# stella-cv/stella_vslam

Hardware: AMD Instinct MI355X
Metric: frames/s ORB-extract+match @640x480,2k kpts (higher is better)
Workload: dtype u8

## Files before the change

stella_vslam_amd/csrc/orb_kernels.hip:

```cpp
#include "svgpu_internal.h"
#include <cstdlib>
#include <utility>

#pragma clang fp contract(off)

namespace {

__device__ __constant__ float c_pattern_f[1024] = {
#include "orb_pattern_i8.inc"
};

__device__ __forceinline__ int find_level(const OrbLevel* __restrict__ L, int num_levels, int idx, int OrbLevel::*first,
                                          int* local) {
    int lv = 0;
    for (int l = 0; l < num_levels; ++l) {
        const int f = L[l].*first;
        if (idx >= f) lv = l;
    }
    *local = idx - L[lv].*first;
    return lv;
}

__device__ __forceinline__ int reflect101(int p, int len) {
    if (len == 1) return 0;
    while (p < 0 || p >= len) p = p < 0 ? -p : 2 * (len - 1) - p;
    return p;
}

typedef unsigned short u16x2 __attribute__((ext_vector_type(2)));
__device__ __forceinline__ u16x2 as_u16x2(uint32_t v) { return __builtin_bit_cast(u16x2, v); }

__device__ __forceinline__ void xcd_frame_map(int per_frame, int batch, int& item, int& frame) {
    const int lin = blockIdx.x + blockIdx.y * gridDim.x;
    const int full = (batch / 8) * 8, lim = full * per_frame;
    if (lin < lim) {
        const int xcd = lin & 7, idx = lin >> 3;
        frame = (idx / per_frame) * 8 + xcd;
        item = idx % per_frame;
    }
    else {
        const int r = lin - lim;
        frame = full + r / per_frame;
        item = r % per_frame;
    }
}

__device__ __forceinline__ void sv_glds16(unsigned long long base, uint32_t voff, uint32_t lds_dst) {
    uint32_t keep;
    asm volatile("s_mov_b32 %0, m0\n\ts_mov_b32 m0, %3\n\ts_nop 2\n\tglobal_load_lds_dwordx4 %1, %2\n\ts_mov_b32 m0, %0"
                 : "=&s"(keep)
                 : "v"(voff), "s"(base), "s"(lds_dst)
                 : "memory");
}

__global__ __launch_bounds__(256) void k_resize(const uint8_t* __restrict__ src, size_t src_frame_stride, int src_pitch,
                                                int sw, uint8_t* __restrict__ dst, size_t dst_frame_stride, int dst_pitch,
                                                int dw, int dh, const short* __restrict__ xofs,
                                                const short2* __restrict__ xa, const short2* __restrict__ yofs,
                                                const short2* __restrict__ yb) {
    const int dy = blockIdx.y * 4 + threadIdx.y;
    const int dx0 = (blockIdx.x * 64 + threadIdx.x) * 4;
    if (dy >= dh || dx0 >= dw) return;
    const uint8_t* S = src + (size_t)blockIdx.z * src_frame_stride;
    const short2 yo = yofs[dy];
    const short2 bb = yb[dy];
    const uint8_t* S0 = S + (size_t)yo.x * src_pitch;
    const uint8_t* S1 = S + (size_t)yo.y * src_pitch;
    uint32_t packed = 0;
#pragma unroll
    for (int i = 0; i < 4; ++i) {
        const int dx = dx0 + i;
        if (dx < dw) {
            const int sx = xofs[dx];
            const short2 a = xa[dx];
            const int sx1 = min(sx + 1, sw - 1);
            const int r0 = S0[sx] * a.x + S0[sx1] * a.y;
            const int r1 = S1[sx] * a.x + S1[sx1] * a.y;
            const int v = ((((int)bb.x * (r0 >> 4)) >> 16) + (((int)bb.y * (r1 >> 4)) >> 16) + 2) >> 2;
            packed |= (uint32_t)(v & 255) << (8 * i);
        }
    }
    uint8_t* D = dst + (size_t)blockIdx.z * dst_frame_stride + (size_t)dy * dst_pitch + dx0;
    *reinterpret_cast<uint32_t*>(D) = packed;
}

#define PYR_THREADS 1024
#define PYR_MAXW 4096
__global__ __launch_bounds__(PYR_THREADS) void k_pyramid(const OrbLevel* __restrict__ L, int num_levels, const int2* __restrict__ band_rows,
                                                         const uint8_t* __restrict__ img0, size_t img0_frame_stride, int img0_pitch,
                                                         uint8_t* __restrict__ pyr, size_t pyr_frame_bytes,
                                                         const short* __restrict__ xofs, const short2* __restrict__ xa,
                                                         const short2* __restrict__ yofs, const short2* __restrict__ yb) {
    __shared__ short s_xo[PYR_MAXW];
    __shared__ short2 s_xa[PYR_MAXW];
    const int band = blockIdx.x, b = blockIdx.y, tid = threadIdx.x;
    uint8_t* P = pyr + (size_t)b * pyr_frame_bytes;
    for (int l = 1; l < num_levels; ++l) {
        const OrbLevel lev = L[l], prev = L[l - 1];
        const uint8_t* S = l == 1 ? img0 + (size_t)b * img0_frame_stride : P + prev.pyr_off;
        const int sp = l == 1 ? img0_pitch : prev.pitch;
        uint8_t* Dst = P + lev.pyr_off;
        const int2 rr = band_rows[band * num_levels + l];
        const int groups = (lev.w + 3) >> 2, ntask = (rr.y - rr.x) * groups;
        const bool in_lds = lev.w <= PYR_MAXW;
        if (in_lds)
            for (int x = tid; x < lev.w; x += PYR_THREADS) {
                s_xo[x] = xofs[lev.xtab_off + x];
                s_xa[x] = xa[lev.xtab_off + x];
            }
        __syncthreads();
        for (int t = tid; t < ntask; t += PYR_THREADS) {
            const int row = t / groups, g = t - row * groups;
            const int dy = rr.x + row, dx0 = g * 4;
            const short2 yo = yofs[lev.ytab_off + dy], bb = yb[lev.ytab_off + dy];
            const uint8_t* S0 = S + (size_t)yo.x * sp;
            const uint8_t* S1 = S + (size_t)yo.y * sp;
            int sx[4], sx1[4];
            short2 a[4];
#pragma unroll
            for (int i = 0; i < 4; ++i) {
                const int dx = min(dx0 + i, lev.w - 1);
                sx[i] = in_lds ? s_xo[dx] : xofs[lev.xtab_off + dx];
                a[i] = in_lds ? s_xa[dx] : xa[lev.xtab_off + dx];
                sx1[i] = min(sx[i] + 1, prev.w - 1);
            }
            int p00[4], p01[4], p10[4], p11[4];
#pragma unroll
            for (int i = 0; i < 4; ++i) {
                p00[i] = S0[sx[i]];
                p01[i] = S0[sx1[i]];
                p10[i] = S1[sx[i]];
                p11[i] = S1[sx1[i]];
            }
            uint32_t packed = 0;
#pragma unroll
            for (int i = 0; i < 4; ++i) {
                const int r0 = p00[i] * a[i].x + p01[i] * a[i].y;
                const int r1 = p10[i] * a[i].x + p11[i] * a[i].y;
                const int v = ((((int)bb.x * (r0 >> 4)) >> 16) + (((int)bb.y * (r1 >> 4)) >> 16) + 2) >> 2;
                packed |= (uint32_t)(v & 255) << (8 * i);
            }
            *reinterpret_cast<uint32_t*>(Dst + (size_t)dy * lev.pitch + dx0) = packed;
        }
        __syncthreads();
    }
}

__device__ __forceinline__ uint32_t mul_hi_u24(uint32_t a, uint32_t b) {
    uint32_t d;
    asm("v_mul_hi_u32_u24 %0, %1, %2" : "=v"(d) : "v"(a), "v"(b));
    return d;
}

__global__ __launch_bounds__(PYR_THREADS) void k_pyramid_lds(const OrbLevel* __restrict__ L, int num_levels, const int2* __restrict__ band_rows,
                                                             int bands, const uint8_t* __restrict__ img0, size_t img0_frame_stride,
                                                             int img0_pitch, uint8_t* __restrict__ pyr, size_t pyr_frame_bytes,
                                                             const uint32_t* __restrict__ xg, const short4* __restrict__ yrow) {
    extern __shared__ __attribute__((aligned(16))) uint8_t s_mem[];
    __shared__ int s_img[SV_MAX_LEVELS], s_yt[SV_MAX_LEVELS + 1];
    const int band = blockIdx.x, b = blockIdx.y, tid = threadIdx.x;
    const int2* BR = band_rows + (size_t)band * num_levels;
    if (tid == 0) {
        int size_a = 0, size_b = 0;
        for (int l = 0; l < num_levels; ++l) {
            const int bytes = (BR[l].y - BR[l].x) * ((L[l].w + 3) & ~3);
            if (l & 1) size_a = max(size_a, bytes);
            else size_b = max(size_b, bytes);
        }
        size_a = (size_a + 15) & ~15;
        size_b = (size_b + 15) & ~15;
        for (int l = 0; l < num_levels; ++l) s_img[l] = (l & 1) ? 0 : size_a;
        int off = size_a + size_b;
        s_yt[0] = off;
        for (int l = 1; l < num_levels; ++l) {
            s_yt[l] = off;
            off += (BR[l].y - BR[l].x) * 8;
        }
        s_yt[num_levels] = off;
    }
    __syncthreads();
    const uint8_t* I0 = img0 + (size_t)b * img0_frame_stride;
    {
        const int w0 = L[0].w, p0 = (w0 + 3) & ~3, lo0 = BR[0].x, n0 = BR[0].y - lo0;
        uint8_t* D0 = s_mem + s_img[0];
        if (((((size_t)I0) | (size_t)img0_pitch) & 15) == 0 && (p0 & 15) == 0) {
            const int cpr = p0 >> 4, total = n0 * cpr;
            const float inv = 1.0f / (float)cpr;
            for (int i = tid; i < total; i += PYR_THREADS) {
                const int r = (int)(((float)i + 0.5f) * inv), c = i - __mul24(r, cpr);
                reinterpret_cast<uint4*>(D0)[i] = *reinterpret_cast<const uint4*>(I0 + (__umul24(lo0 + r, img0_pitch) + 16 * c));
            }
        }
        else if (((((size_t)I0) | (size_t)img0_pitch) & 3) == 0) {
            const int wpr = p0 >> 2, total = n0 * wpr;
            const float inv = 1.0f / (float)wpr;
            for (int i = tid; i < total; i += PYR_THREADS) {
                const int r = (int)(((float)i + 0.5f) * inv), c = i - __mul24(r, wpr);
                reinterpret_cast<uint32_t*>(D0)[i] = *reinterpret_cast<const uint32_t*>(I0 + (__umul24(lo0 + r, img0_pitch) + 4 * c));
            }
        }
        else {
            const int total = n0 * p0;
            for (int i = tid; i < total; i += PYR_THREADS) {
                const int r = i / p0, c = i - r * p0;
                D0[i] = c < w0 ? I0[(size_t)(lo0 + r) * img0_pitch + c] : (uint8_t)0;
            }
        }
        const int rows = (s_yt[num_levels] - s_yt[0]) >> 3;
        for (int i = tid; i < rows; i += PYR_THREADS) {
            int l = 1;
            while (l + 1 < num_levels && s_yt[0] + 8 * i >= s_yt[l + 1]) ++l;
            const int r = i - ((s_yt[l] - s_yt[0]) >> 3);
            reinterpret_cast<short4*>(s_mem + s_yt[0])[i] = yrow[L[l].ytab_off + BR[l].x + r];
        }
    }
    __syncthreads();
    uint8_t* P = pyr + (size_t)b * pyr_frame_bytes;
    for (int l = 1; l < num_levels; ++l) {
        const OrbLevel lev = L[l];
        const int spw = ((L[l - 1].w + 3) & ~3) >> 2, dpw = ((lev.w + 3) & ~3) >> 2;
        const int src_lo = BR[l - 1].x, lo = BR[l].x, hi = BR[l].y;
        const int own_lo = (int)((long long)band * lev.h / bands), own_hi = (int)((long long)(band + 1) * lev.h / bands);
        const uint32_t* S = reinterpret_cast<const uint32_t*>(s_mem + s_img[l - 1]);
        uint32_t* Dl = reinterpret_cast<uint32_t*>(s_mem + s_img[l]);
        const short4* yt = reinterpret_cast<const short4*>(s_mem + s_yt[l]);
        uint8_t* Dg = P + lev.pyr_off;
        const int groups = (lev.w + 3) >> 2, nrows = hi - lo;
        const int chunks = max(min(PYR_THREADS / groups, nrows), 1), rc = (nrows + chunks - 1) / chunks;
        const int c = (int)(((float)tid + 0.5f) * (1.0f / (float)groups)), g = tid - __mul24(c, groups);
        const int r0 = __mul24(c, rc), r1 = min(r0 + rc, nrows);
        if (r0 < r1) {
            const uint4 e = reinterpret_cast<const uint4*>(xg)[2 * (lev.xg_off + g)];
            const uint2 e2 = reinterpret_cast<const uint2*>(xg)[4 * (lev.xg_off + g) + 2];
            const int i0 = e.x & 0xffff, i2 = e.x >> 16;
            const uint32_t coef[4] = {e.z, e.w, e2.x, e2.y};
            uint32_t sel[4];
#pragma unroll
            for (int i = 0; i < 4; ++i) sel[i] = 0x0c010c00u + ((e.y >> (8 * i)) & 255u) * 0x00010001u;
            const uint32_t* S0 = S + (i0 - __mul24(src_lo, spw));
            const int d2 = i2 - i0;
            auto hrow = [&](int sy, uint32_t (&h)[4]) {
                const uint32_t* R = S0 + __mul24(sy, spw);
                const uint32_t a0 = R[0], a1 = R[1], c0 = R[d2], c1 = R[d2 + 1];
                h[0] = __builtin_amdgcn_udot2(as_u16x2(__builtin_amdgcn_perm(a1, a0, sel[0])), as_u16x2(coef[0]), 0u, false) & ~15u;
                h[1] = __builtin_amdgcn_udot2(as_u16x2(__builtin_amdgcn_perm(a1, a0, sel[1])), as_u16x2(coef[1]), 0u, false) & ~15u;
                h[2] = __builtin_amdgcn_udot2(as_u16x2(__builtin_amdgcn_perm(c1, c0, sel[2])), as_u16x2(coef[2]), 0u, false) & ~15u;
                h[3] = __builtin_amdgcn_udot2(as_u16x2(__builtin_amdgcn_perm(c1, c0, sel[3])), as_u16x2(coef[3]), 0u, false) & ~15u;
            };
            uint32_t* dl = Dl + (__mul24(r0, dpw) + g);
            uint32_t goff = __umul24(lo + r0, lev.pitch) + 4 * g;
            const uint32_t own_n = (uint32_t)(own_hi - own_lo);
            uint32_t dyo = (uint32_t)(lo + r0 - own_lo);
            int prev = -1;
            auto step = [&](int row, uint32_t (&top)[4], uint32_t (&bot)[4]) {
                const short4 ye = yt[row];
                if (ye.x != prev) hrow(ye.x, top);
                hrow(ye.y, bot);
                prev = ye.y;
                const uint32_t b0 = (uint32_t)ye.z << 12, b1 = (uint32_t)ye.w << 12;
                uint32_t v[4];
#pragma unroll
                for (int i = 0; i < 4; ++i) v[i] = (mul_hi_u24(b0, top[i]) + mul_hi_u24(b1, bot[i]) + 2u) >> 2;
                const uint32_t packed = (v[0] & 255u) | ((v[1] & 255u) << 8) | ((v[2] & 255u) << 16) | (v[3] << 24);
                *dl = packed;
                if (dyo < own_n) *reinterpret_cast<uint32_t*>(Dg + goff) = packed;
                dl += dpw;
                goff += (uint32_t)lev.pitch;
                ++dyo;
            };
            uint32_t hX[4], hY[4] = {0, 0, 0, 0};
            int row = r0;
            for (; row + 1 < r1; row += 2) {
                step(row, hY, hX);
                step(row + 1, hX, hY);
            }
            if (row < r1) step(row, hY, hX);
        }
        __syncthreads();
    }
}

#define BLUR_EDGE_ROWS 8
struct BlurRow {
    uint32_t w0, w1, w2;
};
enum { BLUR_INTERIOR = 0, BLUR_EDGE = 1, BLUR_GATHER = 2, BLUR_LDS = 3 };
struct BlurEdge {
    bool left, hi_p1;
    uint32_t sel1, sel2;
};
__device__ __forceinline__ uint32_t blur_selector(int xbase, int lo_base, int w) {
    uint32_t s = 0;
#pragma unroll
    for (int k = 0; k < 4; ++k) {
        const int x = xbase + k, sx = x < w ? x : 2 * (w - 1) - x;
        s |= (uint32_t)min(max(sx - lo_base, 0), 7) << (8 * k);
    }
    return s;
}
__device__ __forceinline__ BlurEdge blur_edge_ctx(int x0, int w) {
    BlurEdge e;
    e.left = x0 == 0;
    e.hi_p1 = x0 + 4 < w;
    e.sel1 = blur_selector(x0, x0 - 4, w);
    e.sel2 = blur_selector(x0 + 4, e.hi_p1 ? x0 : x0 - 4, w);
    return e;
}
template <int MODE>
__device__ __forceinline__ BlurRow blur_load(const uint8_t* __restrict__ row, int x0, int w, const BlurEdge& e) {
    BlurRow r;
    if (MODE == BLUR_INTERIOR) {
        const uint32_t* p = reinterpret_cast<const uint32_t*>(row + x0 - 4);
        r.w0 = p[0];
        r.w1 = p[1];
        r.w2 = p[2];
    }
    else if (MODE == BLUR_EDGE) {
        if (e.left) {
            const uint32_t* p = reinterpret_cast<const uint32_t*>(row);
            r.w1 = p[0];
            r.w2 = p[1];
            r.w0 = __builtin_amdgcn_perm(r.w2, r.w1, 0x01020304u);
        }
        else {
            const uint32_t* p = reinterpret_cast<const uint32_t*>(row + x0 - 4);
            const uint32_t pm1 = p[0], p0 = p[1], p1 = e.hi_p1 ? p[2] : 0u;
            r.w0 = pm1;
            r.w1 = __builtin_amdgcn_perm(p0, pm1, e.sel1);
            r.w2 = e.hi_p1 ? __builtin_amdgcn_perm(p1, p0, e.sel2) : __builtin_amdgcn_perm(p0, pm1, e.sel2);
        }
    }
    else {
        uint32_t b[12];
#pragma unroll
        for (int k = 0; k < 12; ++k) b[k] = row[reflect101(x0 - 4 + k, w)];
        r.w0 = b[0] | (b[1] << 8) | (b[2] << 16) | (b[3] << 24);
        r.w1 = b[4] | (b[5] << 8) | (b[6] << 16) | (b[7] << 24);
        r.w2 = b[8] | (b[9] << 8) | (b[10] << 16) | (b[11] << 24);
    }
    return r;
}
__device__ __forceinline__ void blur_hpair(const BlurRow& a, const BlurRow& b, u16x2 (&hp)[4]) {
    u16x2 q[10];
#define SV_PK(WA, WB, K) as_u16x2(__builtin_amdgcn_perm(WB, WA, 0x0c000c00u | ((4u + K) << 16) | K))
    q[0] = SV_PK(a.w0, b.w0, 1u);
    q[1] = SV_PK(a.w0, b.w0, 2u);
    q[2] = SV_PK(a.w0, b.w0, 3u);
    q[3] = SV_PK(a.w1, b.w1, 0u);
    q[4] = SV_PK(a.w1, b.w1, 1u);
    q[5] = SV_PK(a.w1, b.w1, 2u);
    q[6] = SV_PK(a.w1, b.w1, 3u);
    q[7] = SV_PK(a.w2, b.w2, 0u);
    q[8] = SV_PK(a.w2, b.w2, 1u);
    q[9] = SV_PK(a.w2, b.w2, 2u);
#undef SV_PK
    const u16x2 t18 = {18, 18}, t34 = {34, 34}, t48 = {48, 48}, t56 = {56, 56};
#pragma unroll
    for (int j = 0; j < 4; ++j) hp[j] = t18 * (q[j] + q[j + 6]) + t34 * (q[j + 1] + q[j + 5]) + t48 * (q[j + 2] + q[j + 4]) + t56 * q[j + 3];
}
__device__ __forceinline__ uint32_t blur_dot(u16x2 h, uint32_t taps, uint32_t acc) { return __builtin_amdgcn_udot2(h, as_u16x2(taps), acc, false); }
__device__ __forceinline__ uint32_t blur_pack(const uint32_t (&acc)[4]) {
    const uint32_t lo = __builtin_amdgcn_perm(acc[1], acc[0], 0x0c0c0602u), hi = __builtin_amdgcn_perm(acc[3], acc[2], 0x06020c0cu);
    return lo | hi;
}

template <int MODE, class LoadPair>
__device__ __forceinline__ void blur_walk(LoadPair load_pair, uint8_t* __restrict__ Dp, int dpitch, int ys, int ye) {
    constexpr int AHEAD = MODE == BLUR_LDS ? 0 : 2;
    u16x2 A[4], B[4], C[4], D[4], E[4];
    BlurRow n0 = {}, n1 = {};
    {
        BlurRow r[8];
#pragma unroll
        for (int k = 0; k < 4; ++k) load_pair(ys - 4 + 2 * k, r[2 * k], r[2 * k + 1]);
        if (AHEAD) load_pair(ys + 4, n0, n1);
        if (MODE == BLUR_INTERIOR) {
#pragma unroll
            for (int k = 0; k < 8; ++k) asm volatile("" : "+v"(r[k].w0), "+v"(r[k].w1), "+v"(r[k].w2));
            asm volatile("" : "+v"(n0.w0), "+v"(n0.w1), "+v"(n0.w2), "+v"(n1.w0), "+v"(n1.w1), "+v"(n1.w2));
        }
        blur_hpair(r[0], r[1], A);
        blur_hpair(r[2], r[3], B);
        blur_hpair(r[4], r[5], C);
        blur_hpair(r[6], r[7], D);
    }
    for (int y = ys; y < ye; y += 2) {
        const BlurRow c0 = n0, c1 = n1;
        load_pair(y + 4 + AHEAD, n0, n1);
        if (AHEAD) blur_hpair(c0, c1, E);
        else blur_hpair(n0, n1, E);
        uint32_t acc[4];
#pragma unroll
        for (int j = 0; j < 4; ++j)
            acc[j] = blur_dot(D[j], 34u | (18u << 16), blur_dot(C[j], 56u | (48u << 16), blur_dot(B[j], 34u | (48u << 16), blur_dot(A[j], 18u << 16, 32768u))));
        *reinterpret_cast<uint32_t*>(Dp + __umul24(y, dpitch)) = blur_pack(acc);
        if (y + 1 < ye) {
#pragma unroll
            for (int j = 0; j < 4; ++j)
                acc[j] = blur_dot(E[j], 18u, blur_dot(D[j], 48u | (34u << 16), blur_dot(C[j], 48u | (56u << 16), blur_dot(B[j], 18u | (34u << 16), 32768u))));
            *reinterpret_cast<uint32_t*>(Dp + __umul24(y + 1, dpitch)) = blur_pack(acc);
        }
#pragma unroll
        for (int j = 0; j < 4; ++j) {
            A[j] = B[j];
            B[j] = C[j];
            C[j] = D[j];
            D[j] = E[j];
        }
    }
}
template <int MODE>
__device__ __forceinline__ void blur_strip(const uint8_t* __restrict__ src, int spitch, int w, int h, uint8_t* __restrict__ dst,
                                           int dpitch, int x0, int ys, int ye) {
    auto row_ptr = [&](int y) { return src + __umul24(reflect101(y, h), spitch); };
    BlurEdge edge = {};
    if (MODE == BLUR_EDGE) edge = blur_edge_ctx(x0, w);
    blur_walk<MODE>([&](int y, BlurRow& a, BlurRow& b) {
        a = blur_load<MODE>(row_ptr(y), x0, w, edge);
        b = blur_load<MODE>(row_ptr(y + 1), x0, w, edge);
    }, dst + x0, dpitch, ys, ye);
}

__device__ __forceinline__ void blur_locate(const OrbLevel* __restrict__ L, int num_levels, const uint8_t* __restrict__ img0,
                                            size_t img0_frame_stride, int img0_pitch, const uint8_t* __restrict__ pyr,
                                            size_t pyr_frame_bytes, uint8_t* __restrict__ blur, size_t blur_frame_bytes, OrbLevel& lev,
                                            int& tile, const uint8_t*& src, int& spitch, uint8_t*& dst,
                                            int OrbLevel::*first = &OrbLevel::btile_first) {
    int b, item;
    xcd_frame_map(gridDim.x, gridDim.y, item, b);
    const int lv = find_level(L, num_levels, item, first, &tile);
    lev = L[lv];
    if (lv == 0) {
        src = img0 + (size_t)b * img0_frame_stride;
        spitch = img0_pitch;
    }
    else {
        src = pyr + (size_t)b * pyr_frame_bytes + lev.pyr_off;
        spitch = lev.pitch;
    }
    dst = blur + (size_t)b * blur_frame_bytes + lev.blur_off;
}
__device__ __forceinline__ bool blur_streamable(const uint8_t* src, int spitch, int w) {
    return ((((size_t)src) | (size_t)spitch) & 3) == 0 && w >= 16;
}
template <int ROWS>
__global__ __launch_bounds__(256) void k_blur(const OrbLevel* __restrict__ L, int num_levels, const uint8_t* __restrict__ img0,
                                              size_t img0_frame_stride, int img0_pitch, const uint8_t* __restrict__ pyr,
                                              size_t pyr_frame_bytes, uint8_t* __restrict__ blur, size_t blur_frame_bytes) {
    OrbLevel lev;
    int tile, spitch;
    const uint8_t* src;
    uint8_t* dst;
    blur_locate(L, num_levels, img0, img0_frame_stride, img0_pitch, pyr, pyr_frame_bytes, blur, blur_frame_bytes, lev, tile, src, spitch, dst);
    if (!blur_streamable(src, spitch, lev.w)) return;
    const int main_tiles = lev.btiles_x * lev.btiles_y;
    if (tile < main_tiles) {
        const int tx = tile % lev.btiles_x, ty = tile / lev.btiles_x;
        const int rem_groups = tx == lev.btiles_x - 1 ? (min(lev.w - 6, (tx + 1) * BLUR_TW) - tx * BLUR_TW + 3) / 4 : 64;
        int g = 64;
        while (g > 1 && (g >> 1) >= rem_groups) g >>= 1;
        if (g <= 32 && rem_groups > 0) {
            const int spw = 64 / g, lane = threadIdx.x & 63;
            if (ty * spw >= lev.btiles_y) return;
            const int strip = (ty * 4 + (int)(threadIdx.x >> 6)) * spw + lane / g;
            const int x0 = tx * BLUR_TW + (lane % g) * 4, ys = strip * ROWS;
            if (x0 >= lev.w || ys >= lev.h) return;
            if (x0 >= 4 && x0 + 6 < lev.w) blur_strip<BLUR_INTERIOR>(src, spitch, lev.w, lev.h, dst, lev.pitch, x0, ys, min(ys + ROWS, lev.h));
            return;
        }
        const int x0 = tx * BLUR_TW + (threadIdx.x & 63) * 4;
        const int ys = __builtin_amdgcn_readfirstlane(ty * (4 * ROWS) + (int)(threadIdx.x >> 6) * ROWS);
        if (x0 >= lev.w || ys >= lev.h) return;
        if (x0 >= 4 && x0 + 6 < lev.w) blur_strip<BLUR_INTERIOR>(src, spitch, lev.w, lev.h, dst, lev.pitch, x0, ys, min(ys + ROWS, lev.h));
    }
    else {
        const int which = threadIdx.x & 3, strip = (tile - main_tiles) * 64 + (threadIdx.x >> 2);
        const int ys = strip * BLUR_EDGE_ROWS;
        const int last = ((lev.w - 1) >> 2) << 2;
        int x0;
        if (which == 0) x0 = 0;
        else if (which == 1) x0 = last;
        else if (which == 2) x0 = last - 4;
        else return;
        if (ys >= lev.h || x0 < 0 || (which != 0 && (x0 == 0 || x0 + 6 < lev.w))) return;
        blur_strip<BLUR_EDGE>(src, spitch, lev.w, lev.h, dst, lev.pitch, x0, ys, min(ys + BLUR_EDGE_ROWS, lev.h));
    }
}
#define BLUR_LP (16 + BLUR_SEG + 16)
#define BLUR_LDS_ROWS (BLUR_ROWS + 8)
static_assert(BLUR_SEG % 16 == 0 && BLUR_BAND_THREADS % 64 == 0 && BLUR_SEG / 4 <= BLUR_BAND_THREADS && BLUR_ROWS % 2 == 0, "blur band geometry");
static_assert(BLUR_LDS_ROWS * BLUR_LP <= 64 * 1024, "blur band exceeds the static LDS limit");
template <>
__global__ __launch_bounds__(BLUR_BAND_THREADS) void k_blur<BLUR_ROWS>(const OrbLevel* __restrict__ L, int num_levels, const uint8_t* __restrict__ img0,
                                                                       size_t img0_frame_stride, int img0_pitch, const uint8_t* __restrict__ pyr,
                                                                       size_t pyr_frame_bytes, uint8_t* __restrict__ blur, size_t blur_frame_bytes) {
    __shared__ __attribute__((aligned(16))) uint8_t s_rows[BLUR_LDS_ROWS * BLUR_LP];
    OrbLevel lev;
    int item, spitch;
    const uint8_t* src;
    uint8_t* dst;
    blur_locate(L, num_levels, img0, img0_frame_stride, img0_pitch, pyr, pyr_frame_bytes, blur, blur_frame_bytes, lev, item, src, spitch, dst,
                &OrbLevel::bband_first);
    if (!blur_streamable(src, spitch, lev.w)) return;
    const int tid = threadIdx.x, w = lev.w, h = lev.h;
    const int seg = item % lev.bband_segs, xs = seg * BLUR_SEG, sw = min(BLUR_SEG, w - xs);
    const int y0 = (item / lev.bband_segs) * BLUR_ROWS, rows = min(BLUR_ROWS, h - y0);
    const int groups = (sw + 3) >> 2, xend = xs + 4 * groups + 4;
    {
        constexpr int CPR = BLUR_LP / 16;
        const int total = (rows + 6) * CPR;
        const unsigned long long base = (unsigned long long)(uintptr_t)src;
        const uint32_t lds0 = __builtin_amdgcn_readfirstlane((uint32_t)(uintptr_t)(const __attribute__((address_space(3))) uint8_t*)s_rows) + BLUR_LP;
        for (int q0 = __builtin_amdgcn_readfirstlane(tid & ~63); q0 < total; q0 += BLUR_BAND_THREADS) {
            const int q = q0 + (tid & 63), k = q / CPR, x = xs - 16 + 16 * (q - k * CPR);
            if (q < total && x >= 0 && x < min(w, xend)) {
                const uint32_t off = __umul24(reflect101(y0 - 3 + k, h), spitch) + (uint32_t)x;
                if (x + 16 <= w) sv_glds16(base, off, lds0 + 16u * (uint32_t)q0);
                else
#pragma clang loop vectorize(disable)
                    for (int d = 0; x + 4 * d < w; ++d)
                        *reinterpret_cast<uint32_t*>(s_rows + BLUR_LP + 16 * q + 4 * d) = *reinterpret_cast<const uint32_t*>(src + off + 4 * d);
            }
        }
        asm volatile("s_waitcnt vmcnt(0)" ::: "memory");
    }
    __syncthreads();
    for (int i = tid; i < (rows + 6) * 8; i += BLUR_BAND_THREADS) {
        uint8_t* row = s_rows + ((i >> 3) + 1) * BLUR_LP + 16 - xs;
        const int j = i & 7;
        if (j == 0 && xs == 0) {
            const uint32_t* p = reinterpret_cast<const uint32_t*>(row);
            reinterpret_cast<uint32_t*>(row)[-1] = __builtin_amdgcn_perm(p[1], p[0], 0x01020304u);
        }
        const int x = w - 1 + j;
        if (j > 0 && x < xend) row[x] = row[2 * (w - 1) - x];
    }
    __syncthreads();
    const int chunks = max(min(BLUR_BAND_THREADS / groups, rows >> 1), 1), rc = ((rows + chunks - 1) / chunks + 1) & ~1;
    const int c = (int)(((float)tid + 0.5f) * (1.0f / (float)groups)), g = tid - __mul24(c, groups);
    const int r0 = __mul24(c, rc), r1 = min(r0 + rc, rows);
    if (r0 >= r1) return;
    const uint32_t* S = reinterpret_cast<const uint32_t*>(s_rows + 12 + 4 * g);
    blur_walk<BLUR_LDS>([&](int y, BlurRow& a, BlurRow& b) {
        const uint32_t* p = S + __mul24(y + 4, BLUR_LP / 4);
        a = BlurRow{p[0], p[1], p[2]};
        b = BlurRow{p[BLUR_LP / 4], p[BLUR_LP / 4 + 1], p[BLUR_LP / 4 + 2]};
    }, dst + __umul24(y0, lev.pitch) + xs + 4 * g, lev.pitch, r0, r1);
}
template <int ROWS>
__global__ __launch_bounds__(256) void k_blur_gather(const OrbLevel* __restrict__ L, int num_levels, const uint8_t* __restrict__ img0,
                                                     size_t img0_frame_stride, int img0_pitch, const uint8_t* __restrict__ pyr,
                                                     size_t pyr_frame_bytes, uint8_t* __restrict__ blur, size_t blur_frame_bytes) {
    OrbLevel lev;
    int tile, spitch;
    const uint8_t* src;
    uint8_t* dst;
    blur_locate(L, num_levels, img0, img0_frame_stride, img0_pitch, pyr, pyr_frame_bytes, blur, blur_frame_bytes, lev, tile, src, spitch, dst);
    if (blur_streamable(src, spitch, lev.w) || tile >= lev.btiles_x * lev.btiles_y) return;
    const int x0 = (tile % lev.btiles_x) * BLUR_TW + (threadIdx.x & 63) * 4;
    const int ys = (tile / lev.btiles_x) * (4 * ROWS) + (threadIdx.x >> 6) * ROWS;
    if (x0 >= lev.w || ys >= lev.h) return;
    blur_strip<BLUR_GATHER>(src, spitch, lev.w, lev.h, dst, lev.pitch, x0, ys, min(ys + ROWS, lev.h));
}

typedef short s16x2 __attribute__((ext_vector_type(2)));
__device__ __forceinline__ int arc_score16(int v, const int (&p)[16]) {
    s16x2 e[16];
#pragma unroll
    for (int k = 0; k < 16; ++k) e[k] = __builtin_bit_cast(s16x2, __mul24(p[k], -65535) + (int)0xFFFF0000);
    s16x2 m2[8], m4[8];
#pragma unroll
    for (int j = 0; j < 8; ++j) m2[j] = __builtin_elementwise_min(e[2 * j + 1], e[(2 * j + 2) & 15]);
#pragma unroll
    for (int j = 0; j < 8; ++j) m4[j] = __builtin_elementwise_min(m2[j], m2[(j + 1) & 7]);
    s16x2 best = s16x2{(short)-32768, (short)-32768};
#pragma unroll
    for (int j = 0; j < 8; ++j) {
        const s16x2 m8 = __builtin_elementwise_min(m4[j], m4[(j + 2) & 7]);
        best = __builtin_elementwise_max(best, __builtin_elementwise_min(m8, __builtin_elementwise_max(e[2 * j], e[(2 * j + 9) & 15])));
    }
    return max(max((int)best.x - v, v + 1 + (int)best.y), 0);
}

#define FAST_KT 12
#define FP 80
__global__ __launch_bounds__(256) void k_fast(const OrbLevel* __restrict__ L, int num_levels, const FastCell* __restrict__ cells, int num_cells, int cpw,
                                              const uint8_t* __restrict__ img0, size_t img0_frame_stride, int img0_pitch,
                                              const uint8_t* __restrict__ pyr, size_t pyr_frame_bytes,
                                              const unsigned short* __restrict__ gtab, unsigned long long* __restrict__ keys,
                                              int total_grid, int ini_thr, int min_thr, const uint8_t* __restrict__ mask,
                                              size_t mask_frame_stride, int mask_pitch, int mask_w, int mask_h) {
    __shared__ __attribute__((aligned(16))) uint8_t s_raw[SV_ROI_MAX * FP + 16];
    __shared__ __attribute__((aligned(16))) uint8_t s_a[SV_ROI_MAX * FP];
    __shared__ unsigned short s_q[SV_CELL * SV_CELL];
    __shared__ unsigned long long s_key[FAST_KT * FAST_KT];
    __shared__ unsigned short s_gx[SV_ROI_MAX], s_gy[SV_ROI_MAX];
    __shared__ int s_count;
    int b, grp;
    xcd_frame_map(gridDim.x, gridDim.y, grp, b);
    const int tid = threadIdx.x, lane = tid & 63;
    const int wv = __builtin_amdgcn_readfirstlane(tid >> 6);
    const uint8_t* M = mask ? mask + (size_t)b * mask_frame_stride : nullptr;
    const uint8_t* const I0 = img0 + (size_t)b * img0_frame_stride;
    const uint8_t* const PY = pyr + (size_t)b * pyr_frame_bytes;
    unsigned long long* const KF = keys + (size_t)b * total_grid;
    uint8_t* const s_img = s_raw + 3;
    unsigned short* const my_q = s_q + wv * (SV_CELL * SV_CELL / 4);
    const int qrow = lane >> 4, qk = lane & 15;
    const int x0 = 3 + 4 * qk;
    const int ly0 = 3 + 4 * (4 * qrow + wv);
    const int e0 = (ly0 << 7) | x0;
    const uint32_t* const qbase = reinterpret_cast<const uint32_t*>(s_raw + ly0 * FP + 4 * qk);

    auto load_ring = [&](const uint8_t* c, int (&p)[16]) {
        p[0] = c[3 * FP];
        p[1] = c[3 * FP + 1];
        p[2] = c[2 * FP + 2];
        p[3] = c[FP + 3];
        p[4] = c[3];
        p[5] = c[-FP + 3];
        p[6] = c[-2 * FP + 2];
        p[7] = c[-3 * FP + 1];
        p[8] = c[-3 * FP];
        p[9] = c[-3 * FP - 1];
        p[10] = c[-2 * FP - 2];
        p[11] = c[-FP - 3];
        p[12] = c[-3];
        p[13] = c[FP - 3];
        p[14] = c[2 * FP - 2];
        p[15] = c[3 * FP - 1];
    };

    const int c_first = grp * cpw, c_last = min(c_first + cpw, num_cells);
    for (int ci = c_first; ci < c_last; ++ci) {
    const FastCell cell = cells[ci];
    const OrbLevel lev = L[cell.lv];
    auto masked = [&](int y, int x) -> bool {
        int my = (int)((float)y * lev.scale), mx = (int)((float)x * lev.scale);
        my = min(my, mask_h - 1);
        mx = min(mx, mask_w - 1);
        return M[(size_t)my * mask_pitch + mx] == 0;
    };
    if (M) {
        const int y0 = cell.min_y, y1 = cell.min_y + cell.h, xa = cell.min_x, xb = cell.min_x + cell.w;
        if (masked(y0, xa) || masked(y1, xa) || masked(y0, xb) || masked(y1, xb)) continue;
    }
    const uint8_t* src;
    int spitch;
    if (cell.lv == 0) {
        src = I0;
        spitch = img0_pitch;
    }
    else {
        src = PY + lev.pyr_off;
        spitch = lev.pitch;
    }
    const int w = cell.w, h = cell.h;
    if (ci != c_first) __syncthreads();
    const uint8_t* rsrc = src + (size_t)cell.min_y * spitch + (cell.min_x - 3);
    {
        const unsigned long long rbase = (unsigned long long)(uintptr_t)rsrc;
        const uint32_t lds_raw = __builtin_amdgcn_readfirstlane((uint32_t)(uintptr_t)(const __attribute__((address_space(3))) uint8_t*)s_raw) + (uint32_t)wv * 1024u;
#pragma unroll
        for (int it = 0; it < 2; ++it) {
            const int q = tid + 256 * it, r = q / 5, c = q - 5 * r;
            if (it == 0 || wv < 2) {
                if (q < SV_ROI_MAX * (FP / 16) && r < h && 16 * c < w + 3) sv_glds16(rbase, (uint32_t)(__umul24(r, spitch) + 16 * c), lds_raw + 4096u * it);
            }
            if (q < SV_ROI_MAX * (FP / 16)) reinterpret_cast<uint4*>(s_a)[q] = make_uint4(0, 0, 0, 0);
        }
    }
    if (tid == 0) {
        s_count = 0;
    }
    if (tid < FAST_KT * FAST_KT) s_key[tid] = 0ull;
    if (tid < w) s_gx[tid] = gtab[lev.gtab_x_off + cell.min_x + tid - SV_PATCH_RADIUS];
    else if (tid >= 128 && tid - 128 < h) s_gy[tid - 128] = gtab[lev.gtab_y_off + cell.min_y + (tid - 128) - SV_PATCH_RADIUS];
    uint32_t band80 = 0;
#pragma unroll
    for (int j = 0; j < 4; ++j) band80 |= (x0 + j < w - 3) ? (0x80u << (8 * j)) : 0u;
    asm volatile("s_waitcnt vmcnt(0)" ::: "memory");
    __syncthreads();

    unsigned long long* K = KF + lev.grid_first;
    const int gx0 = s_gx[3], gy0 = s_gy[3];
    for (int pass = 0; pass < 2; ++pass) {
    const int t = pass == 0 ? ini_thr : min_thr, tq = t;
    int wq = 0;
#if defined(FAST_ABLATE) && FAST_ABLATE >= 2
    if (mask_h == -12345)
#endif
    {
        const uint32_t tqq = (uint32_t)(tq + 1) * 0x10001u;
        uint32_t m = 0;
#pragma unroll
        for (int g = 0; g < 4; ++g) {
            const uint32_t* const rc = qbase + g * (FP / 4);
            const uint32_t w0 = rc[0], w1 = rc[1], w2 = rc[2], w3 = rc[3];
            const uint32_t d1 = rc[3 * (FP / 4) + 1], d2 = rc[3 * (FP / 4) + 2], u1 = rc[-3 * (FP / 4) + 1], u2 = rc[-3 * (FP / 4) + 2];
            auto pk = [](uint32_t hi, uint32_t lo, uint32_t sel) { return __builtin_bit_cast(s16x2, __builtin_amdgcn_perm(hi, lo, sel)); };
            uint32_t e2[2];
#pragma unroll
            for (int half = 0; half < 2; ++half) {
                const s16x2 v = pk(w2, w1, half ? 0x0c050c04u : 0x0c030c02u);
                const s16x2 p0 = pk(d2, d1, half ? 0x0c050c04u : 0x0c030c02u);
                const s16x2 p8 = pk(u2, u1, half ? 0x0c050c04u : 0x0c030c02u);
                const s16x2 p12 = pk(w1, w0, half ? 0x0c060c05u : 0x0c040c03u);
                const s16x2 p4 = pk(w3, w2, half ? 0x0c040c03u : 0x0c020c01u);
                const s16x2 up = __builtin_elementwise_min(__builtin_elementwise_max(p0, p8), __builtin_elementwise_max(p4, p12));
                const s16x2 dn = __builtin_elementwise_max(__builtin_elementwise_min(p0, p8), __builtin_elementwise_min(p4, p12));
                const s16x2 mm = __builtin_elementwise_max(up - v, v - dn);
                e2[half] = __builtin_bit_cast(uint32_t, mm - __builtin_bit_cast(s16x2, tqq));
            }
            const uint32_t sgn = __builtin_amdgcn_perm(e2[1], e2[0], 0x07050301u);
            m = (m >> 1) | (~sgn & (ly0 + g < h - 3 ? band80 : 0u));
        }
        const int cnt = __popc(m);
        int incl = cnt;
        incl += __builtin_amdgcn_update_dpp(0, incl, 0x111, 0xF, 0xF, false);
        incl += __builtin_amdgcn_update_dpp(0, incl, 0x112, 0xF, 0xF, false);
        incl += __builtin_amdgcn_update_dpp(0, incl, 0x114, 0xF, 0xF, false);
        incl += __builtin_amdgcn_update_dpp(0, incl, 0x118, 0xF, 0xF, false);
        incl += __builtin_amdgcn_update_dpp(0, incl, 0x142, 0xA, 0xF, false);
        incl += __builtin_amdgcn_update_dpp(0, incl, 0x143, 0xC, 0xF, false);
        wq = __builtin_amdgcn_readlane(incl, 63);
        int pos = incl - cnt;
        while (m) {
            const int bit = __ffs((int)m) - 1;
            m &= m - 1;
            my_q[pos++] = (unsigned short)(e0 + (((bit & 7) - 4) << 7) + (bit >> 3));
        }
    }
#if defined(FAST_ABLATE) && FAST_ABLATE >= 1
    if (mask_h != -12345) wq = 0;
#endif
    __builtin_amdgcn_fence(__ATOMIC_RELEASE, "wavefront");
    __builtin_amdgcn_wave_barrier();
    __builtin_amdgcn_fence(__ATOMIC_ACQUIRE, "wavefront");
    for (int i = lane; i < wq; i += 64) {
        const int e = my_q[i], ly = e >> 7, qx = e & 127;
        const uint8_t* c = &s_img[ly * FP + qx];
        int p[16];
        load_ring(c, p);
        s_a[ly * FP + qx] = (uint8_t)arc_score16(c[0], p);
    }
    __syncthreads();

    {
        int found = 0;
        for (int i = lane; i < wq; i += 64) {
            const int e = my_q[i], ly = e >> 7, qx = e & 127;
            const uint8_t* a = &s_a[ly * FP + qx];
            const int A = a[0];
            if (A <= t) continue;
            const int s = A - 1;
            const int n0 = max(max((int)a[-FP - 1], (int)a[-FP]), (int)a[-FP + 1]);
            const int n1 = max(max((int)a[-1], (int)a[1]), (int)a[FP - 1]);
            const int n2 = max(max((int)a[FP], (int)a[FP + 1]), n0);
            const bool keep = A > 1 && max(n1, n2) < A;
            if (!keep) continue;
            ++found;
            const int x_level = cell.min_x + qx, y_level = cell.min_y + ly;
            if (M && masked(y_level, x_level)) continue;
            const int gx = s_gx[qx], gy = s_gy[ly];
            const uint32_t order = (uint32_t)cell.order_base | ((uint32_t)ly << 7) | (uint32_t)qx;
            const unsigned long long key = ((unsigned long long)(uint32_t)s << 32) | (0xFFFFFFFFu - order);
            const int kx = gx - gx0, ky = gy - gy0;
            if ((unsigned)kx < FAST_KT && (unsigned)ky < FAST_KT) atomicMax(&s_key[ky * FAST_KT + kx], key);
            else atomicMax(&K[gy * lev.grid_x + gx], key);
        }
        if (found) atomicAdd(&s_count, found);
        __syncthreads();
        if (s_count > 0) break;
        __syncthreads();
    }
    }
    if (tid < FAST_KT * FAST_KT) {
        const unsigned long long key = s_key[tid];
        if (key) atomicMax(&K[(gy0 + tid / FAST_KT) * lev.grid_x + gx0 + tid % FAST_KT], key);
    }
    }
}

__global__ __launch_bounds__(1024) void k_select(const OrbLevel* __restrict__ L, int num_levels, unsigned long long* __restrict__ keys,
                                                 int total_grid, int4* __restrict__ sel, int32_t* __restrict__ counts, int32_t* __restrict__ cellpos) {
    __shared__ int s_wave[16], s_lvcnt[SV_MAX_LEVELS];
    const int b = blockIdx.x, tid = threadIdx.x, lane = tid & 63, wave = tid >> 6;
    unsigned long long* K = keys + (size_t)b * total_grid;
    int4* S = sel + (size_t)b * total_grid;
    if (tid < SV_MAX_LEVELS) s_lvcnt[tid] = 0;
    int running = 0;
    for (int base = 0; base < total_grid; base += 1024) {
        const int idx = base + tid;
        unsigned long long key = 0;
        if (idx < total_grid) {
            key = K[idx];
            if (key) K[idx] = 0;
        }
        const unsigned long long bal = __ballot(key != 0);
        const int before = __popcll(bal & ((1ull << lane) - 1ull));
        __syncthreads();
        if (lane == 0) s_wave[wave] = __popcll(bal);
        __syncthreads();
        int woff = 0, total = 0;
#pragma unroll
        for (int k = 0; k < 16; ++k) {
            if (k < wave) woff += s_wave[k];
            total += s_wave[k];
        }
        if (cellpos && idx < total_grid) cellpos[(size_t)b * (total_grid + 1) + idx] = running + woff + before;
        if (key) {
            int lv = 0;
            while (lv + 1 < num_levels && idx >= L[lv + 1].grid_first) ++lv;
            const uint32_t order = 0xFFFFFFFFu - (uint32_t)(key & 0xFFFFFFFFu);
            const int lx = order & 127, ly = (order >> 7) & 127, cid = order >> 14;
            const int cells_x = L[lv].cells_x;
            const int ci = cid / cells_x, cj = cid - ci * cells_x;
            int4 r;
            r.x = SV_PATCH_RADIUS + cj * SV_CELL + lx;
            r.y = SV_PATCH_RADIUS + ci * SV_CELL + ly;
            r.z = lv;
            r.w = (int)(key >> 32);
            S[running + woff + before] = r;
            atomicAdd(&s_lvcnt[lv], 1);
        }
        running += total;
    }
    __syncthreads();
    if (tid < num_levels) counts[b * (1 + num_levels) + 1 + tid] = s_lvcnt[tid];
    if (tid == 0) {
        counts[b * (1 + num_levels)] = running;
        if (cellpos) cellpos[(size_t)b * (total_grid + 1) + total_grid] = running;
    }
}

__device__ __forceinline__ float dev_fast_atan2(float y, float x) {
    const float p1 = 0.9997878412794807f * (float)(180 / 3.1415926535897932384626433832795);
    const float p3 = -0.3258083974640975f * (float)(180 / 3.1415926535897932384626433832795);
    const float p5 = 0.1555786518463281f * (float)(180 / 3.1415926535897932384626433832795);
    const float p7 = -0.04432655554792128f * (float)(180 / 3.1415926535897932384626433832795);
    const float eps = (float)2.2204460492503131e-16;
    const float ax = fabsf(x), ay = fabsf(y);
    float a, c, c2;
    if (ax >= ay) {
        c = ay / (ax + eps);
        c2 = c * c;
        a = (((p7 * c2 + p5) * c2 + p3) * c2 + p1) * c;
    }
    else {
        c = ax / (ay + eps);
// ... 507 lines not shown
```

Before: 277,600.

## Compute LDS-banded Gaussian blur with int8 MFMA matrix multiplies

Replaces the per-thread scalar/dot2 separable 7-tap blur in the LDS band kernel with two passes of 32x32x32 int8 MFMA. The horizontal and vertical passes are expressed as multiplies by constant banded tap matrices, which are precomputed in device memory. The horizontal result is split into lo/hi byte planes (signed offset via XOR 0x80 with a folded bias constant) so the second MFMA stays exact. It also adds a waves_per_eu hint. The aim is to move blur arithmetic onto the matrix cores, at the cost of redundant MAC work from the banded matrices, extra perm/packing instructions and more tile-boundary bookkeeping.

```diff
diff --git a/stella_vslam_amd/csrc/orb_kernels.hip b/stella_vslam_amd/csrc/orb_kernels.hip
--- a/stella_vslam_amd/csrc/orb_kernels.hip
+++ b/stella_vslam_amd/csrc/orb_kernels.hip
@@ -284,7 +284,7 @@
 struct BlurRow {
     uint32_t w0, w1, w2;
 };
-enum { BLUR_INTERIOR = 0, BLUR_EDGE = 1, BLUR_GATHER = 2, BLUR_LDS = 3 };
+enum { BLUR_INTERIOR = 0, BLUR_EDGE = 1, BLUR_GATHER = 2 };
 struct BlurEdge {
     bool left, hi_p1;
     uint32_t sel1, sel2;
@@ -366,14 +366,14 @@
 
 template <int MODE, class LoadPair>
 __device__ __forceinline__ void blur_walk(LoadPair load_pair, uint8_t* __restrict__ Dp, int dpitch, int ys, int ye) {
-    constexpr int AHEAD = MODE == BLUR_LDS ? 0 : 2;
+    constexpr int AHEAD = 2;
     u16x2 A[4], B[4], C[4], D[4], E[4];
     BlurRow n0 = {}, n1 = {};
     {
         BlurRow r[8];
 #pragma unroll
         for (int k = 0; k < 4; ++k) load_pair(ys - 4 + 2 * k, r[2 * k], r[2 * k + 1]);
-        if (AHEAD) load_pair(ys + 4, n0, n1);
+        load_pair(ys + 4, n0, n1);
         if (MODE == BLUR_INTERIOR) {
 #pragma unroll
             for (int k = 0; k < 8; ++k) asm volatile("" : "+v"(r[k].w0), "+v"(r[k].w1), "+v"(r[k].w2));
@@ -387,8 +387,7 @@
     for (int y = ys; y < ye; y += 2) {
         const BlurRow c0 = n0, c1 = n1;
         load_pair(y + 4 + AHEAD, n0, n1);
-        if (AHEAD) blur_hpair(c0, c1, E);
-        else blur_hpair(n0, n1, E);
+        blur_hpair(c0, c1, E);
         uint32_t acc[4];
 #pragma unroll
         for (int j = 0; j < 4; ++j)
@@ -490,8 +489,28 @@
 #define BLUR_LDS_ROWS (BLUR_ROWS + 8)
 static_assert(BLUR_SEG % 16 == 0 && BLUR_BAND_THREADS % 64 == 0 && BLUR_SEG / 4 <= BLUR_BAND_THREADS && BLUR_ROWS % 2 == 0, "blur band geometry");
 static_assert(BLUR_LDS_ROWS * BLUR_LP <= 64 * 1024, "blur band exceeds the static LDS limit");
+typedef int v4i __attribute__((ext_vector_type(4)));
+typedef int v16i __attribute__((ext_vector_type(16)));
+#define BLUR_MT_OUT 26
+static_assert(BLUR_ROWS > BLUR_MT_OUT && BLUR_ROWS <= 2 * BLUR_MT_OUT && BLUR_ROWS - BLUR_MT_OUT + 32 < BLUR_LDS_ROWS && BLUR_LP % 32 == 0 && BLUR_SEG + 32 <= BLUR_LP,
+              "blur tile geometry");
+struct alignas(16) BlurMfmaB {
+    uint32_t w[3][64][4];
+};
+constexpr uint32_t blur_tap(int i) { return i == 0 || i == 6 ? 18u : i == 1 || i == 5 ? 34u : i == 2 || i == 4 ? 48u : i == 3 ? 56u : 0u; }
+constexpr BlurMfmaB blur_mfma_b() {
+    BlurMfmaB t = {};
+    for (int lane = 0; lane < 64; ++lane)
+        for (int j = 0; j < 16; ++j) {
+            const int n = lane & 31, h = lane >> 5, yp = (j & 3) + 8 * (j >> 2) + 4 * h;
+            for (int s = 0; s < 2; ++s) t.w[s][lane][j >> 2] |= blur_tap(32 * s + 16 * h + j - 13 - n) << (8 * (j & 3));
+            if (n < BLUR_MT_OUT) t.w[2][lane][j >> 2] |= blur_tap(yp - n) << (8 * (j & 3));
+        }
+    return t;
+}
+__device__ const BlurMfmaB d_blur_mfma_b = blur_mfma_b();
 template <>
-__global__ __launch_bounds__(BLUR_BAND_THREADS) void k_blur<BLUR_ROWS>(const OrbLevel* __restrict__ L, int num_levels, const uint8_t* __restrict__ img0,
+__global__ __launch_bounds__(BLUR_BAND_THREADS) __attribute__((amdgpu_waves_per_eu(4))) void k_blur<BLUR_ROWS>(const OrbLevel* __restrict__ L, int num_levels, const uint8_t* __restrict__ img0,
                                                                        size_t img0_frame_stride, int img0_pitch, const uint8_t* __restrict__ pyr,
                                                                        size_t pyr_frame_bytes, uint8_t* __restrict__ blur, size_t blur_frame_bytes) {
     __shared__ __attribute__((aligned(16))) uint8_t s_rows[BLUR_LDS_ROWS * BLUR_LP];
@@ -503,6 +522,11 @@
                 &OrbLevel::bband_first);
     if (!blur_streamable(src, spitch, lev.w)) return;
     const int tid = threadIdx.x, w = lev.w, h = lev.h;
+    const v4i* const bfrag = reinterpret_cast<const v4i*>(d_blur_mfma_b.w) + (tid & 63);
+    const v4i bh0 = bfrag[0], bh1 = bfrag[64], bv = bfrag[128];
+    v16i kfold;
+#pragma unroll
+    for (int i = 0; i < 16; ++i) kfold[i] = 128 * 256 * 256 + 128 * 256 + 32768;
     const int seg = item % lev.bband_segs, xs = seg * BLUR_SEG, sw = min(BLUR_SEG, w - xs);
     const int y0 = (item / lev.bband_segs) * BLUR_ROWS, rows = min(BLUR_ROWS, h - y0);
     const int groups = (sw + 3) >> 2, xend = xs + 4 * groups + 4;
@@ -536,16 +560,35 @@
         if (j > 0 && x < xend) row[x] = row[2 * (w - 1) - x];
     }
     __syncthreads();
-    const int chunks = max(min(BLUR_BAND_THREADS / groups, rows >> 1), 1), rc = ((rows + chunks - 1) / chunks + 1) & ~1;
-    const int c = (int)(((float)tid + 0.5f) * (1.0f / (float)groups)), g = tid - __mul24(c, groups);
-    const int r0 = __mul24(c, rc), r1 = min(r0 + rc, rows);
-    if (r0 >= r1) return;
-    const uint32_t* S = reinterpret_cast<const uint32_t*>(s_rows + 12 + 4 * g);
-    blur_walk<BLUR_LDS>([&](int y, BlurRow& a, BlurRow& b) {
-        const uint32_t* p = S + __mul24(y + 4, BLUR_LP / 4);
-        a = BlurRow{p[0], p[1], p[2]};
-        b = BlurRow{p[BLUR_LP / 4], p[BLUR_LP / 4 + 1], p[BLUR_LP / 4 + 2]};
-    }, dst + __umul24(y0, lev.pitch) + xs + 4 * g, lev.pitch, r0, r1);
+    const int lane = tid & 63, n = lane & 31, hh = lane >> 5;
+    const int ntc = (4 * groups + 31) >> 5, ntiles = rows > BLUR_MT_OUT ? 2 * ntc : ntc;
+    for (int t = __builtin_amdgcn_readfirstlane(tid >> 6); t < ntiles; t += BLUR_BAND_THREADS / 64) {
+        const int tr = t >= ntc, tc = t - tr * ntc, r0 = tr * (BLUR_ROWS - BLUR_MT_OUT);
+        const v4i* p = reinterpret_cast<const v4i*>(s_rows + (r0 + 1 + n) * BLUR_LP + 32 * tc + 16 * hh);
+        const v4i a0 = p[0] ^ (int)0x80808080, a1 = p[2] ^ (int)0x80808080;
+        v16i acc = __builtin_amdgcn_mfma_i32_32x32x32_i8(a0, bh0, v16i{}, 0, 0, 0);
+        acc = __builtin_amdgcn_mfma_i32_32x32x32_i8(a1, bh1, acc, 0, 0, 0);
+        v4i lo, hi;
+#pragma unroll
+        for (int g = 0; g < 4; ++g) {
+            const uint32_t t01 = __builtin_amdgcn_perm(acc[4 * g + 1], acc[4 * g], 0x05010400u), t23 = __builtin_amdgcn_perm(acc[4 * g + 3], acc[4 * g + 2], 0x05010400u);
+            lo[g] = __builtin_amdgcn_perm(t23, t01, 0x05040100u) ^ 0x80808080u;
+            hi[g] = __builtin_amdgcn_perm(t23, t01, 0x07060302u);
+        }
+        const v16i slo = __builtin_amdgcn_mfma_i32_32x32x32_i8(lo, bv, kfold, 0, 0, 0);
+        const v16i shi = __builtin_amdgcn_mfma_i32_32x32x32_i8(hi, bv, v16i{}, 0, 0, 0);
+        const int y = r0 + n, x0 = 32 * tc + 4 * hh;
+        if (n < BLUR_MT_OUT && y < rows) {
+            uint8_t* const Dp = dst + __umul24(y0 + y, lev.pitch) + xs + x0;
+#pragma unroll
+            for (int g = 0; g < 4; ++g) {
+                uint32_t o[4];
+#pragma unroll
+                for (int e = 0; e < 4; ++e) o[e] = ((uint32_t)shi[4 * g + e] << 8) + (uint32_t)slo[4 * g + e];
+                if (x0 + 8 * g < 4 * groups) *reinterpret_cast<uint32_t*>(Dp + 8 * g) = blur_pack(o);
+            }
+        }
+    }
 }
 template <int ROWS>
 __global__ __launch_bounds__(256) void k_blur_gather(const OrbLevel* __restrict__ L, int num_levels, const uint8_t* __restrict__ img0,
```

Measured after the change: 253,300. 0.913x the previous value.
